# Sanasar1/Learning-Deep-Neural-Network-In-Distributed-Computing-Environment

Measured on AMD Instinct MI355X. Metric: samples/sec (whole node) + DP scaling eff., 3-layer MLP at 1/2/4/8 MI355X, higher is better.
Workload: dtype bf16

## Files before the change

learning-deep-neural-network-in-distributed-computing-environment_amd/csrc/include/ldnn_common.h:

```cpp
#pragma once
#include <hip/hip_runtime.h>
#include <stdint.h>

namespace ldnn {

typedef uint16_t bf16_t;

typedef __bf16 bf16x8 __attribute__((ext_vector_type(8)));
typedef __bf16 bf16x4 __attribute__((ext_vector_type(4)));
typedef float floatx4 __attribute__((ext_vector_type(4)));
typedef float floatx16 __attribute__((ext_vector_type(16)));
typedef uint16_t u16x4 __attribute__((ext_vector_type(4)));
typedef uint16_t u16x8 __attribute__((ext_vector_type(8)));
typedef uint32_t u32x4 __attribute__((ext_vector_type(4)));

constexpr int kWave = 64;
constexpr int kNumXcd = 8;

__device__ __forceinline__ float bf2f(uint16_t b) { return __uint_as_float(((uint32_t)b) << 16); }

__device__ __forceinline__ uint16_t f2bf(float f) { return __builtin_bit_cast(uint16_t, (__bf16)f); }

__device__ __forceinline__ float wave_sum(float v) {
#pragma unroll
  for (int o = 32; o > 0; o >>= 1) v += __shfl_xor(v, o, 64);
  return v;
}
__device__ __forceinline__ float wave_max(float v) {
#pragma unroll
  for (int o = 32; o > 0; o >>= 1) v = fmaxf(v, __shfl_xor(v, o, 64));
  return v;
}

__device__ __forceinline__ int xcd_remap(int bid, int nwg) {
  const int q = nwg / kNumXcd, r = nwg % kNumXcd;
  const int xcd = bid % kNumXcd, idx = bid / kNumXcd;
  const int base = (xcd < r) ? xcd * (q + 1) : r * (q + 1) + (xcd - r) * q;
  return base + idx;
}

}
```

learning-deep-neural-network-in-distributed-computing-environment_amd/csrc/kernels/gemm_q.hip:

```cpp
#include <type_traits>

#include "ldnn_common.h"
#include "ldnn_gemm_tile.h"
#include "ldnn_kernels.h"

namespace ldnn {
namespace {
namespace kq {

constexpr int BM = 256, BN = 256;
constexpr int kThreads = 256;
constexpr int kTile = 256 * BK * 2;
constexpr int kStage = 2 * kTile;
constexpr int kPieces = kTile / 1024 / 4;
constexpr uint32_t kOOB = 0x80000000u;

struct Op {
  const char* base;
  uint32_t bytes;
  uint32_t voff[kPieces];
  int kslot;
  uint32_t kstep;
};

// ... 229 lines not shown
          *dst = ob;
        }
        if constexpr (kMaskOut) {
          uint32_t bits = 0;
#pragma unroll
          for (int q = 0; q < 8; ++q) bits |= (bf2f(ob[q]) > 0.f ? 1u : 0u) << q;
          p.mask_out[(size_t)m * p.ldmask + (n >> 3)] = (uint8_t)bits;
        }
      }
    }
    __builtin_amdgcn_wave_barrier();
  }
  if constexpr ((XF & 128) != 0) reinterpret_cast<uint32_t*>(p.C)[(size_t)blockIdx.x * kThreads + wid * 64 + lane] = xsum;
  if (kSums && p.dbias != nullptr) {
#pragma unroll
    for (int q = 0; q < 8; ++q) {
      float t = cs[q];
      t += __shfl_xor(t, 16, 64);
      t += __shfl_xor(t, 32, 64);
      cs[q] = t;
    }
    if (lane < 16 && nok) {
#pragma unroll
      for (int q = 0; q < 8; ++q) atomicAdd(p.dbias + n + q, cs[q]);
    }
  }
}

template <int EPI>
__device__ __forceinline__ void epilogue_bf16(const GemmParams& p, floatx4 (&acc)[8][8], char* smem, int wid, int mbase,
                                              int nbase, int lane) {
  typedef short s16x2 __attribute__((ext_vector_type(2)));
  typedef __bf16 bf16x2 __attribute__((ext_vector_type(2)));
  constexpr bool kHead = EPI == EPI_BIAS_RELU_HEAD;
  constexpr bool kRelu = EPI == EPI_BIAS_RELU || EPI == EPI_BIAS_RELU_MASK || kHead;
  constexpr bool kBias = kRelu || EPI == EPI_BIAS;
  constexpr bool kMaskIn = EPI == EPI_DRELU_MASK, kMaskOut = EPI == EPI_BIAS_RELU_MASK;
  constexpr bool kSums = EPI == EPI_NONE || kMaskIn;
  const int g = lane >> 4, r16 = lane & 15;
  floatx4 bias[8];
  if constexpr (kBias) {
#pragma unroll
    for (int j = 0; j < 8; ++j) {
      const int n = nbase + j * 16 + 4 * g;
      bias[j] = n < p.N ? *reinterpret_cast<const floatx4*>(p.bias + n) : floatx4{0.f, 0.f, 0.f, 0.f};
    }
  }
  bf16x8 wf[4];
  if constexpr (kHead) {
    const bf16_t* wrow = p.head_w + (size_t)r16 * p.ldhw;
#pragma unroll
    for (int t = 0; t < 4; ++t) {
      const int nlo = nbase + 32 * t + 4 * g, nhi = nlo + 16;
      const bf16x4 zero = {};
      const bf16x4 lo = nlo < p.N ? *reinterpret_cast<const bf16x4*>(wrow + nlo) : zero;
      const bf16x4 hi = nhi < p.N ? *reinterpret_cast<const bf16x4*>(wrow + nhi) : zero;
      wf[t] = bf16x8{lo[0], lo[1], lo[2], lo[3], hi[0], hi[1], hi[2], hi[3]};
    }
  }
  uint32_t hq[8][8][2];
  const s16x2 zero2 = {0, 0};
#pragma unroll
  for (int j = 0; j < 8; ++j)
#pragma unroll
    for (int i = 0; i < 8; ++i) {
      floatx4 v = acc[j][i];
      if constexpr (kBias) v += bias[j];
#pragma unroll
      for (int h = 0; h < 2; ++h) {
        const bf16x2 pb = {(__bf16)v[2 * h], (__bf16)v[2 * h + 1]};
        s16x2 r = __builtin_bit_cast(s16x2, pb);
        if constexpr (kRelu) r = __builtin_elementwise_max(r, zero2);
        hq[j][i][h] = __builtin_bit_cast(uint32_t, r);
      }
    }
  if constexpr (kHead) {
    floatx4 d[8];
#pragma unroll
    for (int i = 0; i < 8; ++i) {
      d[i] = floatx4{0.f, 0.f, 0.f, 0.f};
#pragma unroll
      for (int t = 0; t < 4; ++t) {
        const u32x4 q = {hq[2 * t][i][0], hq[2 * t][i][1], hq[2 * t + 1][i][0], hq[2 * t + 1][i][1]};
        d[i] = __builtin_amdgcn_mfma_f32_16x16x32_bf16(wf[t], __builtin_bit_cast(bf16x8, q), d[i], 0, 0, 0);
      }
    }
    const int wm = wid >> 1, wn = wid & 1;
    floatx4* xch = reinterpret_cast<floatx4*>(smem + (2 * wm) * 32768);
    if (wn == 1) {
#pragma unroll
      for (int i = 0; i < 8; ++i) xch[i * 64 + lane] = d[i];
    }
    barrier();
    if (wn == 0) {
      float* part = p.head_part + (size_t)(nbase / 256) * p.M * 16;
#pragma unroll
      for (int i = 0; i < 8; ++i) {
        const int m = mbase + i * 16 + r16;
        const floatx4 v = d[i] + xch[i * 64 + lane];
        if (m < p.M) *reinterpret_cast<floatx4*>(part + (size_t)m * 16 + 4 * g) = v;
      }
      __builtin_amdgcn_s_waitcnt(0xc07f);
    }
  }
  char* wbuf = smem + wid * 32768;
#pragma unroll
  for (int i = 0; i < 8; ++i)
#pragma unroll
    for (int j = 0; j < 8; ++j) {
      const int row = i * 16 + r16;
      const int chunk = 2 * j + (g >> 1);
      *reinterpret_cast<uint2*>(wbuf + row * 256 + ((chunk ^ (row & 15)) << 4) + (g & 1) * 8) =
          uint2{hq[j][i][0], hq[j][i][1]};
    }
  const int c8 = lane & 15;
  const int n = nbase + c8 * 8;
  const bool nok = n < p.N;
  uint32_t mk[32];
  if constexpr (kMaskIn) {
#pragma unroll
    for (int it = 0; it < 32; ++it) {
      const int m = mbase + it * 4 + (lane >> 4);
      mk[it] = (nok && m < p.M) ? (uint32_t)p.mask_in[(size_t)m * p.ldmask + (n >> 3)] : 0u;
    }
  }
  __builtin_amdgcn_s_waitcnt(0xc07f);
  __builtin_amdgcn_wave_barrier();
  auto rows = [&](auto sums) {
    constexpr bool kS = decltype(sums)::value;
    float cs[8] = {0.f, 0.f, 0.f, 0.f, 0.f, 0.f, 0.f, 0.f};
#pragma unroll
    for (int it = 0; it < 32; ++it) {
      const int row = it * 4 + (lane >> 4);
      const int m = mbase + row;
      u32x4 v = *reinterpret_cast<const u32x4*>(wbuf + row * 256 + ((c8 ^ (row & 15)) << 4));
      if (!(nok && m < p.M)) continue;
      if constexpr (kMaskIn) {
        const uint32_t b = mk[it];
#pragma unroll
        for (int k = 0; k < 4; ++k)
          v[k] &= (((b >> (2 * k)) & 1u) ? 0x0000ffffu : 0u) | (((b >> (2 * k + 1)) & 1u) ? 0xffff0000u : 0u);
      }
      if constexpr (kS) {
#pragma unroll
        for (int k = 0; k < 4; ++k) {
          cs[2 * k] += __uint_as_float(v[k] << 16);
          cs[2 * k + 1] += __uint_as_float(v[k] & 0xffff0000u);
        }
      }
      u32x4* dst = reinterpret_cast<u32x4*>(reinterpret_cast<bf16_t*>(p.C) + (size_t)m * p.ldc + n);
      if (p.variant & 4096) __builtin_nontemporal_store(v, dst);
      else *dst = v;
      if constexpr (kMaskOut) {
        uint32_t bits = 0;
#pragma unroll
        for (int k = 0; k < 4; ++k) {
          bits |= ((v[k] & 0xffffu) != 0u ? 1u : 0u) << (2 * k);
          bits |= ((v[k] >> 16) != 0u ? 1u : 0u) << (2 * k + 1);
        }
        p.mask_out[(size_t)m * p.ldmask + (n >> 3)] = (uint8_t)bits;
      }
    }
    if constexpr (kS) {
#pragma unroll
      for (int q = 0; q < 8; ++q) {
        float t = cs[q];
        t += __shfl_xor(t, 16, 64);
        t += __shfl_xor(t, 32, 64);
        cs[q] = t;
      }
      if (lane < 16 && nok) {
#pragma unroll
        for (int q = 0; q < 8; ++q) atomicAdd(p.dbias + n + q, cs[q]);
      }
    }
  };
  if constexpr (kSums) {
    if (p.dbias != nullptr) rows(std::true_type{});
    else rows(std::false_type{});
  } else {
    rows(std::false_type{});
  }
}

template <bool A_KC, bool B_KC, int EPI, bool OUT_F32, int XF = 0>
__global__ __launch_bounds__(kThreads, 1) void gemm_kernel(GemmParams p) {
  constexpr bool kDma = !(XF & 1), kWait = !(XF & 2), kRead = !(XF & 4);
  constexpr bool kAsm = !(A_KC && B_KC);
  __shared__ __attribute__((aligned(1024))) char smem[2 * kStage];

  const int tid = threadIdx.x;
  const int lane = tid & 63;
  const int wid = __builtin_amdgcn_readfirstlane(tid >> 6);
  const int wm = wid >> 1, wn = wid & 1;
  int m0, n0;
  {
    const int tiles_m = (p.M + BM - 1) / BM, tiles_n = (p.N + BN - 1) / BN;
    const int gsel = (p.variant >> 8) & 15;
    const int G = gsel ? (1 << (gsel - 1)) : 4;
    const int id = xcd_remap(blockIdx.x, tiles_m * tiles_n);
    const int per_group = G * tiles_n;
    const int first_m = (id / per_group) * G;
    const int gsize = min(tiles_m - first_m, G);
    m0 = (first_m + (id % per_group) % gsize) * BM;
    n0 = ((id % per_group) / gsize) * BN;
  }

  const int nk_all = (p.K + BK - 1) / BK;
  const int per = (nk_all + gridDim.y - 1) / gridDim.y;
  const int kt0 = blockIdx.y * per;
  const int nk = max(0, min(nk_all, kt0 + per) - kt0);
  const int kbase = kt0 * BK;

  Op oa, ob;
  init_op<A_KC>(oa, p.A, p.lda, p.M, p.K, m0, wid, lane);
  init_op<B_KC>(ob, p.B, p.ldb, p.N, p.K, n0, wid, lane);

  floatx4 acc[8][8];
#pragma unroll
  for (int j = 0; j < 8; ++j)
#pragma unroll
    for (int i = 0; i < 8; ++i) acc[j][i] = floatx4{0.f, 0.f, 0.f, 0.f};

  const int kend = kbase + nk * BK;
  auto stage = [&](int t, char* dst) {
    const int k0 = kbase + t * BK;
    issue<A_KC>(oa, dst, k0, p.K, kend, wid);
    issue<B_KC>(ob, dst + kTile, k0, p.K, kend, wid);
  };

  bf16x8 fa0[8], fb0[8], fa1[8], fb1[8];
  mma_fence();
  if (nk > 0) {
    stage(0, smem);
    stage(1, smem + kStage);
    asm volatile("s_waitcnt vmcnt(16)" ::: "memory");
    barrier();
    read8<A_KC, kAsm>(fa0, smem, wm * 8, 0, lane);
    read8<B_KC, kAsm>(fb0, smem + kTile, wn * 8, 0, lane);
  }
  for (int t = 0; t < nk; ++t) {
    char* const cur = smem + (t & 1) * kStage;
    char* const nxt = smem + ((t + 1) & 1) * kStage;
    lgkm_all();
    mma(acc, fa0, fb0, [&](int q) {
      const int r = q >> 1;
      if ((kRead || t == 0) && !(q & 1) && r < 16) {
        if (r < 8) fa1[r] = frag<A_KC, kAsm>(cur, wm * 8 + r, 1, lane);
        else fb1[r - 8] = frag<B_KC, kAsm>(cur + kTile, wn * 8 + r - 8, 1, lane);
      }
    });
    if (kWait) asm volatile("s_waitcnt vmcnt(0)" ::: "memory");
    barrier();
    const int k2 = kbase + (t + 2) * BK;
    const __amdgpu_buffer_rsrc_t ra = rsrc_at<A_KC>(oa, k2, kend), rb = rsrc_at<B_KC>(ob, k2, kend);
    const bool killa = A_KC && (k2 + oa.kslot >= p.K), killb = B_KC && (k2 + ob.kslot >= p.K);
    mma(acc, fa1, fb1, [&](int q) {
      if constexpr (XF & 8) {
        const int rr = q >> 1, r = (q - 32) >> 1;
        if (kRead && q < 32 && (q & 1)) {
          if (rr < 8) fa0[rr] = frag<A_KC, kAsm>(nxt, wm * 8 + rr, 0, lane);
          else fb0[rr - 8] = frag<B_KC, kAsm>(nxt + kTile, wn * 8 + rr - 8, 0, lane);
        }
        if (kDma && q >= 32 && !(q & 1)) {
          if (r < 8) dma1<XF>(ra, cur, oa, r, killa, wid);
          else dma1<XF>(rb, cur + kTile, ob, r - 8, killb, wid);
        }
      } else if constexpr (XF & 16) {
        const int r = q >> 1, rr = (q - 32) >> 1;
        if (kDma && q < 32 && !(q & 1)) {
          if (r < 8) dma1<XF>(ra, cur, oa, r, killa, wid);
          else dma1<XF>(rb, cur + kTile, ob, r - 8, killb, wid);
        }
        if (kRead && q >= 32 && (q & 1)) {
          if (rr < 8) fa0[rr] = frag<A_KC, kAsm>(nxt, wm * 8 + rr, 0, lane);
          else fb0[rr - 8] = frag<B_KC, kAsm>(nxt + kTile, wn * 8 + rr - 8, 0, lane);
        }
      } else {
        const int r = q >> 2;
        if (kDma && !(q & 3)) {
          if (r < 8) dma1<XF>(ra, cur, oa, r, killa, wid);
          else dma1<XF>(rb, cur + kTile, ob, r - 8, killb, wid);
        }
        const int rr = q >> 1;
        if (kRead && (q & 1) && rr < 16) {
          if (rr < 8) fa0[rr] = frag<A_KC, kAsm>(nxt, wm * 8 + rr, 0, lane);
          else fb0[rr - 8] = frag<B_KC, kAsm>(nxt + kTile, wn * 8 + rr - 8, 0, lane);
        }
      }
    });
  }
  mma_fence();

  GemmParams pe = p;
  if (gridDim.y > 1) {
    if (p.c_split_stride > 0) {
      pe.C = reinterpret_cast<char*>(p.C) + (size_t)blockIdx.y * (size_t)p.c_split_stride * (OUT_F32 ? 4u : 2u);
    } else if (!splitk_combine<8, 8, kThreads>(acc, p.ws, p.cnt, blockIdx.x, gridDim.y, blockIdx.y, smem)) {
      return;
    }
  }
  if constexpr ((XF & 64) != 0) {
    float t = 0.f;
#pragma unroll
    for (int j = 0; j < 8; ++j)
#pragma unroll
      for (int i = 0; i < 8; ++i) t += acc[j][i][0] + acc[j][i][3];
    reinterpret_cast<float*>(p.C)[(size_t)blockIdx.x * kThreads + tid] = t;
    return;
  }
  if constexpr (EPI != EPI_OPT_SGD && EPI != EPI_OPT_ADAM) {
    barrier();
// ... 118 lines not shown
```

learning-deep-neural-network-in-distributed-computing-environment_amd/csrc/kernels/head.hip:

```cpp
#include <algorithm>

#include <cstdlib>

#include "ldnn_common.h"
#include "ldnn_gemm_tile.h"
#include "ldnn_kernels.h"

namespace ldnn {

namespace {

constexpr int kFwdWaves = 8;

constexpr int kHeadDgradMaxK = 4096;

__device__ __forceinline__ int hs_off(int r, int q, int K) {
  return r * ((K + 127) & ~127) * 2 + ((q ^ (r & 15)) << 4);
}

template <int NT, bool DG>
__device__ __forceinline__ void head_softmax_xent(const HeadParams& p, floatx4 (&acc)[NT], floatx4 (*red)[NT][64],
                                                  int nred, float* dls, int lane, int row, int slot) {
#pragma unroll
  for (int j = 0; j < NT; ++j)
    for (int q = 0; q < nred; ++q) acc[j] += red[q][j][lane];

  const bool rok = row < p.B;
  const int cb = 4 * (lane >> 4);
  float x[NT][4];
  float mx = -INFINITY;
  int am = 0x7fffffff;
#pragma unroll
  for (int j = 0; j < NT; ++j) {
    const floatx4 bias = *reinterpret_cast<const floatx4*>(p.bias + j * 16 + cb);
#pragma unroll
    for (int r = 0; r < 4; ++r) {
      const int c = j * 16 + cb + r;
      x[j][r] = bf2f(f2bf(acc[j][r] + bias[r]));
      if (c < p.C && x[j][r] > mx) { mx = x[j][r]; am = c; }
    }
  }
#pragma unroll
  for (int o = 16; o <= 32; o <<= 1) {
    const float omx = __shfl_xor(mx, o, 64);
    const int oam = __shfl_xor(am, o, 64);
    if (omx > mx || (omx == mx && oam < am)) { mx = omx; am = oam; }
  }
  const int lab = rok ? (int)p.labels[row] : -1;
  float se = 0.f, xl = 0.f;
#pragma unroll
  for (int j = 0; j < NT; ++j)
#pragma unroll
    for (int r = 0; r < 4; ++r) {
      const int c = j * 16 + cb + r;
      if (c < p.C) {
        const float e = __expf(x[j][r] - mx);
        if (c == lab) xl = x[j][r];
        x[j][r] = e;
        se += e;
      }
    }
  se += __shfl_xor(se, 16, 64);
  se += __shfl_xor(se, 32, 64);
  xl += __shfl_xor(xl, 16, 64);
  xl += __shfl_xor(xl, 32, 64);
  const float inv = 1.f / se;
  if (rok) {
#pragma unroll
    for (int j = 0; j < NT; ++j) {
      const int c0 = j * 16 + cb;
      if (c0 >= p.ld) continue;
      u16x4 lo, g;
#pragma unroll
      for (int r = 0; r < 4; ++r) {
        const int c = c0 + r;
        const float logit = acc[j][r] + *(p.bias + c);
        lo[r] = f2bf(logit);
        g[r] = c < p.C ? f2bf((x[j][r] * inv - (c == lab ? 1.f : 0.f)) * p.grad_scale) : (uint16_t)0;
      }
      if (p.logits) *reinterpret_cast<u16x4*>(p.logits + (size_t)row * p.ld + c0) = lo;
      *reinterpret_cast<u16x4*>(p.dlogits + (size_t)row * p.ld + c0) = g;
    }
  }
  if constexpr (DG) {
    __builtin_amdgcn_s_waitcnt(0xc07f);
    __builtin_amdgcn_wave_barrier();
#pragma unroll
    for (int j = 0; j < NT; ++j) {
      const int c0 = j * 16 + 4 * (lane >> 4);
#pragma unroll
      for (int r = 0; r < 4; ++r) {
        const int c = c0 + r;
        const float gv = (rok && c < p.C) ? bf2f(f2bf((x[j][r] * inv - (c == lab ? 1.f : 0.f)) * p.grad_scale)) : 0.f;
        dls[(lane & 15) * p.ld + c] = gv;
      }
    }
  }
  float loss = (rok && lane < 16) ? (mx + __logf(se) - xl) : 0.f;
  float corr = (rok && lane < 16 && am == lab) ? 1.f : 0.f;
#pragma unroll
  for (int o = 1; o < 16; o <<= 1) {
    loss += __shfl_xor(loss, o, 64);
    corr += __shfl_xor(corr, o, 64);
  }
  if (lane == 0) {
    p.stats[2 * slot] += loss;
    p.stats[2 * slot + 1] += corr;
  }
}

template <int DEPI, bool HS>
__device__ __forceinline__ void head_dgrad_rows(const HeadParams& p, const char* hs, const float* dls, int m0) {
  const int nq = p.K >> 3;
  const int rows = min(16, p.B - m0);
  for (int q = threadIdx.x; q < nq; q += kFwdWaves * 64) {
    float acc[16][8];
#pragma unroll
    for (int r = 0; r < 16; ++r)
#pragma unroll
      for (int i = 0; i < 8; ++i) acc[r][i] = 0.f;
    for (int c = 0; c < p.C; ++c) {
      const u16x8 wv = *reinterpret_cast<const u16x8*>(p.W + (size_t)c * p.ldw + 8 * q);
      float wf[8];
#pragma unroll
      for (int i = 0; i < 8; ++i) wf[i] = bf2f(wv[i]);
#pragma unroll
      for (int r = 0; r < 16; ++r) {
        const float g = dls[r * p.ld + c];
#pragma unroll
        for (int i = 0; i < 8; ++i) acc[r][i] = fmaf(g, wf[i], acc[r][i]);
      }
    }
    float cs[8] = {};
#pragma unroll
    for (int r = 0; r < 16; ++r) {
      if (r >= rows) continue;
      const u16x8 hv = HS ? *reinterpret_cast<const u16x8*>(hs + hs_off(r, q, p.K))
                          : *reinterpret_cast<const u16x8*>(p.h + (size_t)(m0 + r) * p.ldh + 8 * q);
      u16x8 o;
#pragma unroll
      for (int i = 0; i < 8; ++i) {
        const float hf = bf2f(hv[i]);
        float v = acc[r][i];
        if constexpr (DEPI == EPI_DRELU) v = hf > 0.f ? v : 0.f;
        else if constexpr (DEPI == EPI_DSIGMOID) v *= hf * (1.f - hf);
        o[i] = f2bf(v);
        cs[i] += bf2f(o[i]);
      }
      *reinterpret_cast<u16x8*>(p.dh + (size_t)(m0 + r) * p.lddh + 8 * q) = o;
    }
    if (p.dbias != nullptr) {
      float* dst = p.dbias_ws + (size_t)blockIdx.x * p.K + 8 * q;
      reinterpret_cast<floatx4*>(dst)[0] = floatx4{cs[0], cs[1], cs[2], cs[3]};
// ... 196 lines not shown
        else p.db[n] = v;
      }
    }
  }
}

template <int DEPI>
__global__ __launch_bounds__(256) void head_dgrad_stream_kernel(HeadParams p, int rows_per_block) {
  __shared__ float part[8][256];
  const int cg = threadIdx.x & 31, ty = threadIdx.x >> 5;
  const int c0 = (blockIdx.x * 32 + cg) * 8;
  const int r_begin = blockIdx.y * rows_per_block;
  const int r_end = min(p.B, r_begin + rows_per_block);
  const bool cok = c0 < p.K;
  float wf[16][8];
#pragma unroll
  for (int c = 0; c < 16; ++c) {
    u16x8 w = {};
    if (cok && c < p.ldw_rows) w = *reinterpret_cast<const u16x8*>(p.W + (size_t)c * p.ldw + c0);
#pragma unroll
    for (int i = 0; i < 8; ++i) wf[c][i] = bf2f(w[i]);
  }
  float s[8] = {0.f, 0.f, 0.f, 0.f, 0.f, 0.f, 0.f, 0.f};
  auto row_out = [&](const u16x8& g0, const u16x8& g1, const u16x8& hv, int r) {
    float v[8] = {0.f, 0.f, 0.f, 0.f, 0.f, 0.f, 0.f, 0.f};
#pragma unroll
    for (int c = 0; c < 16; ++c) {
      const float gc = bf2f(c < 8 ? g0[c] : g1[c - 8]);
#pragma unroll
      for (int i = 0; i < 8; ++i) v[i] = fmaf(gc, wf[c][i], v[i]);
    }
    u16x8 o;
#pragma unroll
    for (int i = 0; i < 8; ++i) {
      const float hf = bf2f(hv[i]);
      float x = v[i];
      if constexpr (DEPI == EPI_DRELU) x = hf > 0.f ? x : 0.f;
      else if constexpr (DEPI == EPI_DSIGMOID) x *= hf * (1.f - hf);
      o[i] = f2bf(x);
      s[i] += bf2f(o[i]);
    }
    *reinterpret_cast<u16x8*>(p.dh + (size_t)r * p.lddh + c0) = o;
  };
  auto hrow = [&](int r) -> u16x8 { return *reinterpret_cast<const u16x8*>(p.h + (size_t)r * p.ldh + c0); };
  if (cok) {
    int r = r_begin + ty;
    for (; r + 8 < r_end; r += 16) {
      const u16x8* gp0 = reinterpret_cast<const u16x8*>(p.dlogits + (size_t)r * p.ld);
      const u16x8* gp1 = reinterpret_cast<const u16x8*>(p.dlogits + (size_t)(r + 8) * p.ld);
      const u16x8 a0 = gp0[0], a1 = gp0[1], b0 = gp1[0], b1 = gp1[1];
      const u16x8 h0 = hrow(r), h1 = hrow(r + 8);
      row_out(a0, a1, h0, r);
      row_out(b0, b1, h1, r + 8);
    }
    for (; r < r_end; r += 8) {
      const u16x8* gp0 = reinterpret_cast<const u16x8*>(p.dlogits + (size_t)r * p.ld);
      row_out(gp0[0], gp0[1], hrow(r), r);
    }
  }
  if (p.dbias == nullptr) return;
#pragma unroll
  for (int j = 0; j < 8; ++j) part[ty][cg * 8 + j] = s[j];
  __syncthreads();
  if (ty == 0 && cok) {
#pragma unroll
    for (int j = 0; j < 8; ++j) {
      float t = 0.f;
#pragma unroll
      for (int q = 0; q < 8; ++q) t += part[q][cg * 8 + j];
      atomicAdd(p.dbias + c0 + j, t);
    }
  }
}

template <int DEPI>
hipError_t launch_head_dgrad_stream(const HeadParams& p, hipStream_t s) {
  const int gx = (p.K + 255) / 256;
  int gy = (p.B + 255) / 256;
  if (gy > 256) gy = 256;
  const int rpb = (p.B + gy - 1) / gy;
  head_dgrad_stream_kernel<DEPI><<<dim3(gx, gy), 256, 0, s>>>(p, rpb);
  return hipGetLastError();
}

template <int DEPI, bool HS>
hipError_t launch_head_fwd(const HeadParams& p, hipStream_t s) {
  const dim3 grid((p.B + 15) / 16), block(kFwdWaves * 64);
  switch (p.ld / 16) {
    case 1: head_fwd_xent_kernel<1, DEPI, HS><<<grid, block, 0, s>>>(p); break;
    case 2: head_fwd_xent_kernel<2, DEPI, HS><<<grid, block, 0, s>>>(p); break;
    case 3: head_fwd_xent_kernel<3, DEPI, HS><<<grid, block, 0, s>>>(p); break;
    default: head_fwd_xent_kernel<4, DEPI, HS><<<grid, block, 0, s>>>(p); break;
  }
  return hipGetLastError();
}

template <int DEPI>
hipError_t launch_head_fwd_dg(const HeadParams& p, hipStream_t s) {
  return p.dgrad_mode == 2 ? launch_head_fwd<DEPI, true>(p, s) : launch_head_fwd<DEPI, false>(p, s);
}

template <int DEPI>
hipError_t head_dgrad_dispatch(const HeadParams& p, hipStream_t s) {
  if (p.dgrad_mode == 0) {
    hipError_t e = launch_head_fwd<-1, false>(p, s);
    if (e != hipSuccess) return e;
    return launch_head_dgrad_stream<DEPI>(p, s);
  }
  hipError_t e = launch_head_fwd_dg<DEPI>(p, s);
  if (e != hipSuccess || p.dbias == nullptr) return e;
  return slab_sum(p.dbias_ws, p.dbias, p.K / 4, (p.B + 15) / 16, 1.f, s);
}

}

hipError_t head_fwd_xent(const HeadParams& p, hipStream_t s) {
  if (p.B <= 0) return hipSuccess;
  if (p.ld > 64 || p.ld % 16 != 0 || p.C > p.ld || p.ldw_rows > p.ld || p.K % 8 != 0) return hipErrorInvalidValue;
  if (p.dh == nullptr) return launch_head_fwd<-1, false>(p, s);
  if (p.lddh % 8 != 0) return hipErrorInvalidValue;
  if (p.dgrad_mode < 0 || p.dgrad_mode > 2 || (p.dgrad_mode == 0 && p.ld != 16)) return hipErrorInvalidValue;
  if ((p.dgrad_mode == 1 || p.dgrad_mode == 2) &&
      (p.K > kHeadDgradMaxK || (p.dbias != nullptr && p.dbias_ws == nullptr)))
    return hipErrorInvalidValue;
  switch (p.dgrad_epi) {
    case EPI_NONE: return head_dgrad_dispatch<EPI_NONE>(p, s);
    case EPI_DRELU: return head_dgrad_dispatch<EPI_DRELU>(p, s);
    case EPI_DSIGMOID: return head_dgrad_dispatch<EPI_DSIGMOID>(p, s);
    default: return hipErrorInvalidValue;
  }
}

hipError_t head_xent_parts(const HeadParams& p, const float* parts, int nparts, hipStream_t s) {
  if (p.B <= 0) return hipSuccess;
  if (p.ld != 16 || p.C > 16 || nparts < 1 || parts == nullptr) return hipErrorInvalidValue;
  const int slots = (p.B + 15) / 16;
  head_xent_parts_kernel<<<(slots + kPartWaves - 1) / kPartWaves, kPartWaves * 64, 0, s>>>(p, parts, nparts);
  return hipGetLastError();
}

hipError_t head_dgrad_stream(const HeadParams& p, hipStream_t s) {
  if (p.B <= 0) return hipSuccess;
  if (p.ld != 16 || p.dh == nullptr || p.lddh % 8 != 0 || p.K % 8 != 0 || p.ldw_rows > 16) return hipErrorInvalidValue;
  switch (p.dgrad_epi) {
    case EPI_NONE: return launch_head_dgrad_stream<EPI_NONE>(p, s);
    case EPI_DRELU: return launch_head_dgrad_stream<EPI_DRELU>(p, s);
    case EPI_DSIGMOID: return launch_head_dgrad_stream<EPI_DSIGMOID>(p, s);
    default: return hipErrorInvalidValue;
  }
}

typedef short s16x4 __attribute__((ext_vector_type(4)));
constexpr int kHbUnroll = 4;

template <bool RELU>
__global__ __launch_bounds__(256) void head_bwd_kernel(HeadParams p, int rows_per_wg) {
  constexpr int kH = 16 * 128, kD = 16 * 32, kSt = kH + kD;
  constexpr int kWave = kHbUnroll * kSt;
  __shared__ __attribute__((aligned(16))) char smem[4 * kWave];
  static_assert(4 * kWave >= 4 * 64 * 17 * 4, "the reduction scratch fits");
  const int lane = threadIdx.x & 63, wid = threadIdx.x >> 6;
  const int g = lane >> 4, r16 = lane & 15;
  const int n0 = blockIdx.x * 64;
  const int r_begin = blockIdx.y * rows_per_wg, r_end = min(p.B, r_begin + rows_per_wg);
  char* const st = smem + wid * kWave;
  typedef __attribute__((address_space(3))) bf16x4 lds_b4;

  s16x4 wa[4];
#pragma unroll
  for (int t = 0; t < 4; ++t) {
    const int n = n0 + (t >> 1) * 32 + 8 * (r16 >> 2) + (t & 1) * 4 + (r16 & 3);
#pragma unroll
    for (int q = 0; q < 4; ++q) {
      const int c = 4 * g + q;
      wa[t][q] = (c < p.ldw_rows && n < p.K) ? (short)p.W[(size_t)c * p.ldw + n] : (short)0;
    }
  }
  floatx4 acc2[4];
#pragma unroll
  for (int t = 0; t < 4; ++t) acc2[t] = floatx4{0.f, 0.f, 0.f, 0.f};
  float cs[16];
#pragma unroll
  for (int k = 0; k < 16; ++k) cs[k] = 0.f;
  float dbs[4] = {0.f, 0.f, 0.f, 0.f};
  const int q = r16 >> 2, pp = r16 & 3;

  for (int mb = r_begin + wid * 16; mb < r_end; mb += 64 * kHbUnroll) {
    u16x8 hv[kHbUnroll][2];
    uint2 dl[kHbUnroll];
#pragma unroll
    for (int u = 0; u < kHbUnroll; ++u) {
      const int m = mb + u * 64 + r16;
      hv[u][0] = hv[u][1] = u16x8{0, 0, 0, 0, 0, 0, 0, 0};
      dl[u] = uint2{0u, 0u};
      if (m < r_end) {
        const bf16_t* hr = p.h + (size_t)m * p.ldh + n0 + 8 * g;
        hv[u][0] = *reinterpret_cast<const u16x8*>(hr);
        hv[u][1] = *reinterpret_cast<const u16x8*>(hr + 32);
        dl[u] = *reinterpret_cast<const uint2*>(p.dlogits + (size_t)m * 16 + 4 * g);
      }
    }
#pragma unroll
    for (int u = 0; u < kHbUnroll; ++u) {
      char* sb = st + u * kSt;
      *reinterpret_cast<u16x8*>(sb + r16 * 128 + ((g ^ (r16 & 7)) << 4)) = hv[u][0];
      *reinterpret_cast<u16x8*>(sb + r16 * 128 + (((4 + g) ^ (r16 & 7)) << 4)) = hv[u][1];
      *reinterpret_cast<uint2*>(sb + kH + r16 * 32 + ((g ^ ((r16 >> 2) & 3)) << 3)) = dl[u];
    }
#pragma unroll
    for (int u = 0; u < kHbUnroll; ++u) {
      const int m = mb + u * 64 + r16;
      const s16x4 bl = __builtin_bit_cast(s16x4, dl[u]);
      floatx4 d[4];
#pragma unroll
      for (int t = 0; t < 4; ++t)
        d[t] = __builtin_amdgcn_mfma_f32_16x16x16bf16_1k(wa[t], bl, floatx4{0.f, 0.f, 0.f, 0.f}, 0, 0, 0);
      u16x8 o[2];
#pragma unroll
      for (int k = 0; k < 16; ++k) {
        const uint16_t hb = hv[u][k >> 3][k & 7];
        float v = d[k >> 2][k & 3];
        if constexpr (RELU) v = (short)hb > 0 ? v : 0.f;
        const uint16_t ob = f2bf(v);
        o[k >> 3][k & 7] = ob;
        cs[k] += bf2f(ob);
      }
      if (m < r_end) {
        bf16_t* dst = p.dh + (size_t)m * p.lddh + n0 + 8 * g;
        *reinterpret_cast<u16x8*>(dst) = o[0];
        *reinterpret_cast<u16x8*>(dst + 32) = o[1];
      }
#pragma unroll
      for (int c = 0; c < 4; ++c) dbs[c] += bf2f((uint16_t)((c < 2 ? dl[u].x : dl[u].y) >> (16 * (c & 1))));
    }
    __builtin_amdgcn_s_waitcnt(0xc07f);
    __builtin_amdgcn_wave_barrier();
#pragma unroll
    for (int u = 0; u < kHbUnroll; ++u) {
      const char* sb = st + u * kSt;
      const int row = 4 * g + q;
      const bf16x4 bd = __builtin_amdgcn_ds_read_tr16_b64_v4bf16((lds_b4*)(sb + kH + row * 32 + ((pp ^ g) << 3)));
#pragma unroll
      for (int nt = 0; nt < 4; ++nt) {
        const bf16x4 ah = __builtin_amdgcn_ds_read_tr16_b64_v4bf16(
            (lds_b4*)(sb + row * 128 + (((2 * nt + (pp >> 1)) ^ (row & 7)) << 4) + (pp & 1) * 8));
        acc2[nt] = __builtin_amdgcn_mfma_f32_16x16x16bf16_1k(__builtin_bit_cast(s16x4, ah),
                                                             __builtin_bit_cast(s16x4, bd), acc2[nt], 0, 0, 0);
      }
    }
  }

#pragma unroll
  for (int k = 0; k < 16; ++k)
#pragma unroll
    for (int o = 1; o < 16; o <<= 1) cs[k] += __shfl_xor(cs[k], o, 64);
#pragma unroll
  for (int q = 0; q < 4; ++q)
#pragma unroll
    for (int o = 1; o < 16; o <<= 1) dbs[q] += __shfl_xor(dbs[q], o, 64);
  __syncthreads();
  float* red = reinterpret_cast<float*>(smem);
#pragma unroll
  for (int nt = 0; nt < 4; ++nt)
#pragma unroll
    for (int r = 0; r < 4; ++r) red[(wid * 64 + lane) * 17 + nt * 4 + r] = acc2[nt][r];
  __syncthreads();
  if (wid == 0) {
#pragma unroll
    for (int nt = 0; nt < 4; ++nt)
#pragma unroll
      for (int r = 0; r < 4; ++r) {
        float t = 0.f;
#pragma unroll
        for (int w = 0; w < 4; ++w) t += red[(w * 64 + lane) * 17 + nt * 4 + r];
        const int n = n0 + 16 * nt + 4 * g + r;
        if (r16 < p.nrows_w && n < p.K) atomicAdd(p.dW + (size_t)r16 * p.lddw + n, t);
      }
  }
  __syncthreads();
  if (r16 == 0) {
#pragma unroll
    for (int k = 0; k < 16; ++k) red[(wid * 4 + g) * 17 + k] = cs[k];
    red[(wid * 4 + g) * 17 + 16] = 0.f;
#pragma unroll
    for (int q = 0; q < 4; ++q) red[16 * 17 + (wid * 4 + g) * 4 + q] = dbs[q];
  }
  __syncthreads();
  if (threadIdx.x < 64) {
    const int gg = threadIdx.x >> 4, k = threadIdx.x & 15;
    const int n = n0 + (k >> 3) * 32 + 8 * gg + (k & 7);
    if (p.dbias != nullptr && n < p.K) {
      float t = 0.f;
#pragma unroll
      for (int w = 0; w < 4; ++w) t += red[(w * 4 + gg) * 17 + k];
      atomicAdd(p.dbias + n, t);
    }
  } else if (threadIdx.x < 80 && blockIdx.x == 0 && p.db != nullptr) {
    const int c = threadIdx.x - 64, gg = c >> 2, q = c & 3;
    if (c < p.nrows_w) {
      float t = 0.f;
#pragma unroll
      for (int w = 0; w < 4; ++w) t += red[16 * 17 + (w * 4 + gg) * 4 + q];
      atomicAdd(p.db + c, t);
    }
  }
}

hipError_t head_bwd(const HeadParams& p, hipStream_t s) {
  if (p.B <= 0) return hipSuccess;
  if (p.ld != 16 || p.dh == nullptr || p.dW == nullptr || p.lddh % 8 != 0 || p.ldh % 8 != 0 || p.K % 64 != 0 ||
      p.ldw_rows > 16 || p.nrows_w > 16 || (p.dgrad_epi != EPI_NONE && p.dgrad_epi != EPI_DRELU))
    return hipErrorInvalidValue;
  const int gx = p.K / 64;
  constexpr int target = 768;
  int gy = std::max(1, std::min(256, target / gx));
  int rpw = (p.B + gy - 1) / gy;
  rpw = (rpw + 63) & ~63;
  gy = (p.B + rpw - 1) / rpw;
  const dim3 grid(gx, gy);
  if (p.dgrad_epi == EPI_DRELU) head_bwd_kernel<true><<<grid, 256, 0, s>>>(p, rpw);
  else head_bwd_kernel<false><<<grid, 256, 0, s>>>(p, rpw);
  return hipGetLastError();
}

size_t head_dgrad_ws_floats(int B, int K) { return (size_t)((B + 15) / 16) * K; }

int head_dgrad_max_k() { return kHeadDgradMaxK; }

int head_wgrad_splits(int B, int K) {
  const int cols = (K + kWgCols - 1) / kWgCols;
  int s = (256 + cols - 1) / cols;
  const int max_by_rows = B / (kWgWaves * kWgRows * 2);
  if (s > max_by_rows) s = max_by_rows;
  return s < 1 ? 1 : (s > 64 ? 64 : s);
}

hipError_t head_wgrad(const HeadWgradParams& p, int splits, hipStream_t s) {
  if (p.B <= 0 || p.K <= 0) return hipSuccess;
  if (p.ld > 64 || p.ld % 16 != 0 || p.nrows > p.ld || p.K % 8 != 0 || p.ldh % 8 != 0) return hipErrorInvalidValue;
  if (splits < 1) splits = head_wgrad_splits(p.B, p.K);
  const dim3 grid((p.K + kWgCols - 1) / kWgCols, splits), block(kWgWaves * 64);
  switch (p.ld / 16) {
    case 1: head_wgrad_kernel<1><<<grid, block, 0, s>>>(p); break;
    case 2: head_wgrad_kernel<2><<<grid, block, 0, s>>>(p); break;
    case 3: head_wgrad_kernel<3><<<grid, block, 0, s>>>(p); break;
    default: head_wgrad_kernel<4><<<grid, block, 0, s>>>(p); break;
  }
  return hipGetLastError();
}

}
```

Before: 10.36 million.

## Restructure head backward so each wave owns a column block, with prefetch and packed ReLU masks

In head_bwd, each wave now owns its own 64-column slice instead of the four waves of a block splitting rows over the same columns. This removes the cross-wave LDS reduction and its __syncthreads, and each wave issues its own dW/dbias atomics. Row tiles are loaded one iteration ahead into double-buffered registers, full tiles skip bounds checks, the ReLU mask and bf16 packing use packed 16-bit instructions, and the db sum runs only for the first column block. The GEMM mask-out epilogue also uses packed min ops, and the grid and launch bounds are retuned. The cost is higher register pressure and more global atomics per workgroup.

```diff
diff --git a/learning-deep-neural-network-in-distributed-computing-environment_amd/csrc/include/ldnn_common.h b/learning-deep-neural-network-in-distributed-computing-environment_amd/csrc/include/ldnn_common.h
--- a/learning-deep-neural-network-in-distributed-computing-environment_amd/csrc/include/ldnn_common.h
+++ b/learning-deep-neural-network-in-distributed-computing-environment_amd/csrc/include/ldnn_common.h
@@ -21,6 +21,25 @@
 
 __device__ __forceinline__ uint16_t f2bf(float f) { return __builtin_bit_cast(uint16_t, (__bf16)f); }
 
+__device__ __forceinline__ uint32_t pk_max_i16(uint32_t a, uint32_t b) {
+  uint32_t r;
+  asm("v_pk_max_i16 %0, %1, %2" : "=v"(r) : "v"(a), "v"(b));
+  return r;
+}
+__device__ __forceinline__ uint32_t pk_min_u16(uint32_t a, uint32_t b) {
+  uint32_t r;
+  asm("v_pk_min_u16 %0, %1, %2" : "=v"(r) : "v"(a), "v"(b));
+  return r;
+}
+__device__ __forceinline__ uint32_t pk_sub_i16(uint32_t a, uint32_t b) {
+  uint32_t r;
+  asm("v_pk_sub_i16 %0, %1, %2" : "=v"(r) : "v"(a), "v"(b));
+  return r;
+}
+__device__ __forceinline__ uint32_t pk_gt0_mask_i16(uint32_t h) {
+  return pk_sub_i16(0u, pk_min_u16(pk_max_i16(h, 0u), 0x00010001u));
+}
+
 __device__ __forceinline__ float wave_sum(float v) {
 #pragma unroll
   for (int o = 32; o > 0; o >>= 1) v += __shfl_xor(v, o, 64);
diff --git a/learning-deep-neural-network-in-distributed-computing-environment_amd/csrc/kernels/gemm_q.hip b/learning-deep-neural-network-in-distributed-computing-environment_amd/csrc/kernels/gemm_q.hip
--- a/learning-deep-neural-network-in-distributed-computing-environment_amd/csrc/kernels/gemm_q.hip
+++ b/learning-deep-neural-network-in-distributed-computing-environment_amd/csrc/kernels/gemm_q.hip
@@ -405,12 +405,10 @@
       if (p.variant & 4096) __builtin_nontemporal_store(v, dst);
       else *dst = v;
       if constexpr (kMaskOut) {
-        uint32_t bits = 0;
-#pragma unroll
-        for (int k = 0; k < 4; ++k) {
-          bits |= ((v[k] & 0xffffu) != 0u ? 1u : 0u) << (2 * k);
-          bits |= ((v[k] >> 16) != 0u ? 1u : 0u) << (2 * k + 1);
-        }
+        uint32_t bits = pk_min_u16(v[0], 0x00010001u);
+#pragma unroll
+        for (int k = 1; k < 4; ++k) bits |= pk_min_u16(v[k], 0x00010001u) << (2 * k);
+        bits |= bits >> 15;
         p.mask_out[(size_t)m * p.ldmask + (n >> 3)] = (uint8_t)bits;
       }
     }
diff --git a/learning-deep-neural-network-in-distributed-computing-environment_amd/csrc/kernels/head.hip b/learning-deep-neural-network-in-distributed-computing-environment_amd/csrc/kernels/head.hip
--- a/learning-deep-neural-network-in-distributed-computing-environment_amd/csrc/kernels/head.hip
+++ b/learning-deep-neural-network-in-distributed-computing-environment_amd/csrc/kernels/head.hip
@@ -1,4 +1,5 @@
 #include <algorithm>
+#include <type_traits>
 
 #include <cstdlib>
 
@@ -501,17 +502,20 @@
 
 typedef short s16x4 __attribute__((ext_vector_type(4)));
 constexpr int kHbUnroll = 4;
+constexpr int kHbRows = 16 * kHbUnroll;
 
 template <bool RELU>
-__global__ __launch_bounds__(256) void head_bwd_kernel(HeadParams p, int rows_per_wg) {
+__global__ __launch_bounds__(256, 2) void head_bwd_kernel(HeadParams p, int rows_per_wg) {
+  typedef __bf16 bf16x2 __attribute__((ext_vector_type(2)));
   constexpr int kH = 16 * 128, kD = 16 * 32, kSt = kH + kD;
   constexpr int kWave = kHbUnroll * kSt;
   __shared__ __attribute__((aligned(16))) char smem[4 * kWave];
-  static_assert(4 * kWave >= 4 * 64 * 17 * 4, "the reduction scratch fits");
   const int lane = threadIdx.x & 63, wid = threadIdx.x >> 6;
   const int g = lane >> 4, r16 = lane & 15;
-  const int n0 = blockIdx.x * 64;
+  const int n0 = (blockIdx.x * 4 + wid) * 64;
+  if (n0 >= p.K) return;
   const int r_begin = blockIdx.y * rows_per_wg, r_end = min(p.B, r_begin + rows_per_wg);
+  const bool do_db = p.db != nullptr && n0 == 0;
   char* const st = smem + wid * kWave;
   typedef __attribute__((address_space(3))) bf16x4 lds_b4;
 
@@ -534,21 +538,27 @@
   float dbs[4] = {0.f, 0.f, 0.f, 0.f};
   const int q = r16 >> 2, pp = r16 & 3;
 
-  for (int mb = r_begin + wid * 16; mb < r_end; mb += 64 * kHbUnroll) {
-    u16x8 hv[kHbUnroll][2];
-    uint2 dl[kHbUnroll];
+  const int nfull = (r_end - r_begin) / kHbRows;
+  auto row0 = [&](int it) { return r_begin + it * kHbRows; };
+  auto load = [&](auto full, int it, u16x8 (&hv)[kHbUnroll][2], uint2 (&dl)[kHbUnroll]) {
+    const int mb = row0(it);
 #pragma unroll
     for (int u = 0; u < kHbUnroll; ++u) {
-      const int m = mb + u * 64 + r16;
+      const int m = mb + u * 16 + r16;
       hv[u][0] = hv[u][1] = u16x8{0, 0, 0, 0, 0, 0, 0, 0};
       dl[u] = uint2{0u, 0u};
-      if (m < r_end) {
+      if (decltype(full)::value || m < r_end) {
         const bf16_t* hr = p.h + (size_t)m * p.ldh + n0 + 8 * g;
         hv[u][0] = *reinterpret_cast<const u16x8*>(hr);
         hv[u][1] = *reinterpret_cast<const u16x8*>(hr + 32);
         dl[u] = *reinterpret_cast<const uint2*>(p.dlogits + (size_t)m * 16 + 4 * g);
       }
     }
+  };
+  auto iter = [&](auto full, int it, u16x8 (&hv)[kHbUnroll][2], uint2 (&dl)[kHbUnroll],
+                  u16x8 (&hvn)[kHbUnroll][2], uint2 (&dln)[kHbUnroll]) {
+    const int mb = row0(it);
+    if (decltype(full)::value && it + 1 < nfull) load(full, it + 1, hvn, dln);
 #pragma unroll
     for (int u = 0; u < kHbUnroll; ++u) {
       char* sb = st + u * kSt;
@@ -558,29 +568,33 @@
     }
 #pragma unroll
     for (int u = 0; u < kHbUnroll; ++u) {
-      const int m = mb + u * 64 + r16;
+      const int m = mb + u * 16 + r16;
       const s16x4 bl = __builtin_bit_cast(s16x4, dl[u]);
       floatx4 d[4];
 #pragma unroll
       for (int t = 0; t < 4; ++t)
         d[t] = __builtin_amdgcn_mfma_f32_16x16x16bf16_1k(wa[t], bl, floatx4{0.f, 0.f, 0.f, 0.f}, 0, 0, 0);
-      u16x8 o[2];
-#pragma unroll
-      for (int k = 0; k < 16; ++k) {
-        const uint16_t hb = hv[u][k >> 3][k & 7];
-        float v = d[k >> 2][k & 3];
-        if constexpr (RELU) v = (short)hb > 0 ? v : 0.f;
-        const uint16_t ob = f2bf(v);
-        o[k >> 3][k & 7] = ob;
-        cs[k] += bf2f(ob);
-      }
-      if (m < r_end) {
+      const u32x4 hw[2] = {__builtin_bit_cast(u32x4, hv[u][0]), __builtin_bit_cast(u32x4, hv[u][1])};
+      u32x4 o[2];
+#pragma unroll
+      for (int kk = 0; kk < 8; ++kk) {
+        const int k = 2 * kk;
+        const bf16x2 pb = {(__bf16)d[k >> 2][k & 3], (__bf16)d[k >> 2][(k & 3) + 1]};
+        uint32_t ob = __builtin_bit_cast(uint32_t, pb);
+        if constexpr (RELU) ob &= pk_gt0_mask_i16(hw[kk >> 2][kk & 3]);
+        o[kk >> 2][kk & 3] = ob;
+        cs[k] += __uint_as_float(ob << 16);
+        cs[k + 1] += __uint_as_float(ob & 0xffff0000u);
+      }
+      if (decltype(full)::value || m < r_end) {
         bf16_t* dst = p.dh + (size_t)m * p.lddh + n0 + 8 * g;
-        *reinterpret_cast<u16x8*>(dst) = o[0];
-        *reinterpret_cast<u16x8*>(dst + 32) = o[1];
-      }
-#pragma unroll
-      for (int c = 0; c < 4; ++c) dbs[c] += bf2f((uint16_t)((c < 2 ? dl[u].x : dl[u].y) >> (16 * (c & 1))));
+        *reinterpret_cast<u32x4*>(dst) = o[0];
+        *reinterpret_cast<u32x4*>(dst + 32) = o[1];
+      }
+      if (do_db) {
+#pragma unroll
+        for (int c = 0; c < 4; ++c) dbs[c] += bf2f((uint16_t)((c < 2 ? dl[u].x : dl[u].y) >> (16 * (c & 1))));
+      }
     }
     __builtin_amdgcn_s_waitcnt(0xc07f);
     __builtin_amdgcn_wave_barrier();
@@ -597,60 +611,46 @@
                                                              __builtin_bit_cast(s16x4, bd), acc2[nt], 0, 0, 0);
       }
     }
-  }
-
-#pragma unroll
-  for (int k = 0; k < 16; ++k)
-#pragma unroll
-    for (int o = 1; o < 16; o <<= 1) cs[k] += __shfl_xor(cs[k], o, 64);
-#pragma unroll
-  for (int q = 0; q < 4; ++q)
-#pragma unroll
-    for (int o = 1; o < 16; o <<= 1) dbs[q] += __shfl_xor(dbs[q], o, 64);
-  __syncthreads();
-  float* red = reinterpret_cast<float*>(smem);
-#pragma unroll
-  for (int nt = 0; nt < 4; ++nt)
-#pragma unroll
-    for (int r = 0; r < 4; ++r) red[(wid * 64 + lane) * 17 + nt * 4 + r] = acc2[nt][r];
-  __syncthreads();
-  if (wid == 0) {
-#pragma unroll
-    for (int nt = 0; nt < 4; ++nt)
-#pragma unroll
-      for (int r = 0; r < 4; ++r) {
-        float t = 0.f;
-#pragma unroll
-        for (int w = 0; w < 4; ++w) t += red[(w * 64 + lane) * 17 + nt * 4 + r];
-        const int n = n0 + 16 * nt + 4 * g + r;
-        if (r16 < p.nrows_w && n < p.K) atomicAdd(p.dW + (size_t)r16 * p.lddw + n, t);
-      }
-  }
-  __syncthreads();
-  if (r16 == 0) {
-#pragma unroll
-    for (int k = 0; k < 16; ++k) red[(wid * 4 + g) * 17 + k] = cs[k];
-    red[(wid * 4 + g) * 17 + 16] = 0.f;
-#pragma unroll
-    for (int q = 0; q < 4; ++q) red[16 * 17 + (wid * 4 + g) * 4 + q] = dbs[q];
-  }
-  __syncthreads();
-  if (threadIdx.x < 64) {
-    const int gg = threadIdx.x >> 4, k = threadIdx.x & 15;
-    const int n = n0 + (k >> 3) * 32 + 8 * gg + (k & 7);
-    if (p.dbias != nullptr && n < p.K) {
-      float t = 0.f;
-#pragma unroll
-      for (int w = 0; w < 4; ++w) t += red[(w * 4 + gg) * 17 + k];
-      atomicAdd(p.dbias + n, t);
-    }
-  } else if (threadIdx.x < 80 && blockIdx.x == 0 && p.db != nullptr) {
-    const int c = threadIdx.x - 64, gg = c >> 2, q = c & 3;
-    if (c < p.nrows_w) {
-      float t = 0.f;
-#pragma unroll
-      for (int w = 0; w < 4; ++w) t += red[16 * 17 + (w * 4 + gg) * 4 + q];
-      atomicAdd(p.db + c, t);
+  };
+  u16x8 hva[kHbUnroll][2], hvb[kHbUnroll][2];
+  uint2 dla[kHbUnroll], dlb[kHbUnroll];
+  if (nfull > 0) load(std::true_type{}, 0, hva, dla);
+  for (int it = 0; it < nfull; it += 2) {
+    iter(std::true_type{}, it, hva, dla, hvb, dlb);
+    if (it + 1 < nfull) iter(std::true_type{}, it + 1, hvb, dlb, hva, dla);
+  }
+  if (r_begin + nfull * kHbRows < r_end) {
+    load(std::false_type{}, nfull, hva, dla);
+    iter(std::false_type{}, nfull, hva, dla, hvb, dlb);
+  }
+
+  constexpr int kTs = 68;
+  static_assert(2 * 16 * kTs * 4 <= kWave, "the output tiles fit the staging slice");
+  float* const tw = reinterpret_cast<float*>(st);
+  float* const tc = tw + 16 * kTs;
+#pragma unroll
+  for (int nt = 0; nt < 4; ++nt) *reinterpret_cast<floatx4*>(tw + r16 * kTs + 16 * nt + 4 * g) = acc2[nt];
+  if (p.dbias != nullptr) {
+#pragma unroll
+    for (int k = 0; k < 16; k += 4)
+      *reinterpret_cast<floatx4*>(tc + r16 * kTs + (k >> 3) * 32 + 8 * g + (k & 7)) =
+          floatx4{cs[k], cs[k + 1], cs[k + 2], cs[k + 3]};
+  }
+  __builtin_amdgcn_s_waitcnt(0xc07f);
+  __builtin_amdgcn_wave_barrier();
+  for (int c = 0; c < p.nrows_w; ++c) atomicAdd(p.dW + (size_t)c * p.lddw + n0 + lane, tw[c * kTs + lane]);
+  if (p.dbias != nullptr) {
+    float t = 0.f;
+#pragma unroll
+    for (int r = 0; r < 16; ++r) t += tc[r * kTs + lane];
+    atomicAdd(p.dbias + n0 + lane, t);
+  }
+  if (do_db) {
+#pragma unroll
+    for (int c = 0; c < 4; ++c) {
+#pragma unroll
+      for (int o = 1; o < 16; o <<= 1) dbs[c] += __shfl_xor(dbs[c], o, 64);
+      if (r16 == 0 && 4 * g + c < p.nrows_w) atomicAdd(p.db + 4 * g + c, dbs[c]);
     }
   }
 }
@@ -660,11 +660,11 @@
   if (p.ld != 16 || p.dh == nullptr || p.dW == nullptr || p.lddh % 8 != 0 || p.ldh % 8 != 0 || p.K % 64 != 0 ||
       p.ldw_rows > 16 || p.nrows_w > 16 || (p.dgrad_epi != EPI_NONE && p.dgrad_epi != EPI_DRELU))
     return hipErrorInvalidValue;
-  const int gx = p.K / 64;
-  constexpr int target = 768;
+  const int gx = (p.K + 255) / 256;
+  constexpr int target = 512;
   int gy = std::max(1, std::min(256, target / gx));
   int rpw = (p.B + gy - 1) / gy;
-  rpw = (rpw + 63) & ~63;
+  rpw = (rpw + kHbRows - 1) / kHbRows * kHbRows;
   gy = (p.B + rpw - 1) / rpw;
   const dim3 grid(gx, gy);
   if (p.dgrad_epi == EPI_DRELU) head_bwd_kernel<true><<<grid, 256, 0, s>>>(p, rpw);
```

After: 10.38 million (median of 2 runs). Within noise of the previous version (+0.2%).
